# RobinChen121/Stochastic-Inventory

Hardware: NVIDIA B200
Metric: state-action-demand evaluations/s (fp64), full-horizon SDP solve (higher is better)
Workload: dtype f64

## Files before the change

stochastic-inventory_b200/csrc/kernel_lead.cuh:

```cuda
#pragma once
#include <cuda_runtime.h>

#include <cstdlib>

#include "dev_model.cuh"
#include "kernel_tiled.cuh"

namespace sdpb {

constexpr int kLeadYT = 4;

struct LeadArgs {
    int t, D, pmf_off;
    const double* Vn;
    double* Vt;
    int* Qt;
    long long lo, hi;
    long long row0;
    int NYT;
    int ny_tiles, nq2_tiles;
    int A, Apad, di_max, NR;
    int nthreads;
};

__device__ __forceinline__ long long lds_s64(unsigned shared_addr) {
    long long v;
    asm volatile("ld.shared.s64 %0, [%1];" : "=l"(v) : "r"(shared_addr));
    return v;
}

__device__ __forceinline__ double ldg_at(const char* base, long long byte_off) {
    return __ldg(reinterpret_cast<const double*>(base + byte_off));
}

__device__ __forceinline__ double lds_double(unsigned shared_addr) {
    double v;
    asm volatile("ld.shared.f64 %0, [%1];" : "=d"(v) : "r"(shared_addr));
    return v;
}

template <bool IS_MIN, bool LAST, int RQ, bool DEDUP>
__global__ void __launch_bounds__(256)
bi_lead_slab(const __grid_constant__ DevModel M, const __grid_constant__ LeadArgs a) {
    constexpr int YT = kLeadYT;
    extern __shared__ __align__(16) unsigned char smem_raw[];
    const int NYB = YT * a.NYT;
    const int D = a.D, A = a.A, Apad = a.Apad;
    double* slab = reinterpret_cast<double*>(smem_raw);
    const size_t slab_elems = (size_t)max(a.NR, NYB) * RQ * Apad;
    double* Lw = slab + slab_elems;
    double2* PP = reinterpret_cast<double2*>(Lw + ((a.NR + 1) & ~1));

    long long b = blockIdx.x;
    int q2_0 = 0;
    if (M.lead == 2) { q2_0 = (int)(b % a.nq2_tiles) * RQ; b /= a.nq2_tiles; }
    const int ytile = (int)(b % a.ny_tiles); b /= a.ny_tiles;
    const long long ix = DEDUP ? 0 : a.row0 + b;
    const int q1_0 = ytile * NYB;
    const long long y0 = ix + q1_0;
    const int n_levels = DEDUP ? (M.nI + M.nQ - 1) : M.nQ;

    const int tid = threadIdx.x;
    for (int j = tid; j < D; j += a.nthreads) PP[j] = make_double2(M.pmf_p[a.pmf_off + j], M.pmf_pg[a.pmf_off + j]);
    const bool lost = (M.flags & SDPB_F_LOST_SALES) != 0;
    const long long strideX = (M.lead == 2) ? (long long)M.nQ * M.nQ : (long long)M.nQ;
    for (int wi = tid; wi < a.NR; wi += a.nthreads) {
        const double lvl = M.inv_min + (double)(y0 - a.di_max + wi) * M.step;
        Lw[wi] = M.h * fmax(lvl, 0.0) + M.pen * fmax(-lvl, 0.0);
    }
    if (!LAST) {
// ... 382 lines not shown
    if (mn) { if (last) SDPB_COL_LAUNCH(true, true) else SDPB_COL_LAUNCH(true, false) }
    else    { if (last) SDPB_COL_LAUNCH(false, true) else SDPB_COL_LAUNCH(false, false) }
#undef SDPB_COL_LAUNCH
    if (e != cudaSuccess || cudaGetLastError() != cudaSuccess) return SDPB_ERR_CUDA;
    return SDPB_OK;
}

struct DevPeer { char* base0; unsigned long long stride; long long lo, hi; };

template <bool IS_MIN>
__global__ void __launch_bounds__(256)
merge_action_slices(const double* __restrict__ sv, const int* __restrict__ sa, int parts, long long n_local,
                    double* __restrict__ Vt, int* __restrict__ Qt, long long lo, const DevPeer* __restrict__ peers,
                    int n_peers, int t) {
    const long long i = (long long)blockIdx.x * blockDim.x + threadIdx.x;
    if (i >= n_local) return;
    double best = IS_MIN ? DBL_MAX : -DBL_MAX;
    int arg = kNoAction;
    for (int q = 0; q < parts; q++) {
        const double v = sv[(long long)q * n_local + i];
        const int av = sa[(long long)q * n_local + i];
        if (av != kNoAction && (IS_MIN ? (v < best) : (v > best))) { best = v; arg = av; }
    }
    Vt[i] = best;
    Qt[i] = arg == kNoAction ? -1 : arg;
    const long long idx = lo + i;
    for (int p = 0; p < n_peers; p++) {
        const DevPeer pr = peers[p];
        if (idx >= pr.lo && idx < pr.hi)
            reinterpret_cast<double*>(pr.base0 + (unsigned long long)(t - 1) * pr.stride)[idx] = best;
    }
}

struct Q2Args {
    int t, D, pmf_off;
    const double* VnT;
    double* Vt;
    int* Qt;
    long long lo, hi;
    long long f_begin, f_end;
    int n_chunks, tpx;
    int cs;
    double* slice_v;
    int* slice_a;
    int di_max, NRW;
    int parts;
    int n_peer;
    double* peer_v[2];
    long long peer_lo[2], peer_hi[2];
};

struct PeerStore { double* v; long long lo, hi; };

constexpr int kQ2YT = 8, kQ2PF = 2, kQ2PAD = kQ2PF + 1;

__global__ void transpose_q2a(const double* __restrict__ V, double* __restrict__ VT, int nQ, int row0) {
    __shared__ double tile[32][33];
    const long long base = (long long)(row0 + blockIdx.x) * nQ * nQ;
    const int c0 = blockIdx.y * 32, r0 = blockIdx.z * 32;
    for (int r = threadIdx.y; r < 32; r += 8) {
        const int row = r0 + r, c = c0 + threadIdx.x;
        if (row < nQ && c < nQ) tile[r][threadIdx.x] = V[base + (long long)row * nQ + c];
    }
    __syncthreads();
    for (int r = threadIdx.y; r < 32; r += 8) {
        const int row = c0 + r, c = r0 + threadIdx.x;
        if (row < nQ && c < nQ) VT[base + (long long)row * nQ + c] = tile[threadIdx.x][r];
    }
}

template <bool IS_MIN, bool LAST, int NT, int PARTS>
__global__ void __launch_bounds__(NT, 512 / NT)
bi_lead_q2(const __grid_constant__ DevModel M, const __grid_constant__ Q2Args a) {
    constexpr int YT = kQ2YT, PF = kQ2PF, W = YT + PF, PAD = kQ2PAD;
    extern __shared__ __align__(16) unsigned char smem_raw[];
    double2* WR = reinterpret_cast<double2*>(smem_raw);
    double2* PP = WR + a.NRW;
    const int D = a.D, nQ = M.nQ, tid = threadIdx.x;
    constexpr int cols = NT / PARTS;
    const int part = tid / cols, col = tid - part * cols;
    double* MV = reinterpret_cast<double*>(PP + D);
    int* MA = reinterpret_cast<int*>(MV + (size_t)(PARTS - 1) * YT * cols);
    const long long F0 = a.f_begin + (long long)blockIdx.x * cols;
    const long long x_first = F0 / a.tpx;
    const bool lost = (M.flags & SDPB_F_LOST_SALES) != 0;

    for (int j = tid; j < D; j += NT) PP[j] = make_double2(M.pmf_p[a.pmf_off + j], M.pmf_pg[a.pmf_off + j]);
    for (int wi = tid; wi < a.NRW; wi += NT) {
        const long long il = x_first - a.di_max - PAD + wi;
        const double lvl = M.inv_min + (double)il * M.step;
        long long is = il;
        if (lost) is = is > M.i_zero ? is : M.i_zero;
        is = is < M.nI - 1 ? is : M.nI - 1;
        is = is > 0 ? is : 0;
        WR[wi] = make_double2(M.h * fmax(lvl, 0.0) + M.pen * fmax(-lvl, 0.0),
// ... 78 lines not shown
        if (part > 0 || !any) return;
        for (int q = 0; q < PARTS - 1; q++) {
#pragma unroll
            for (int k = 0; k < YT; k++) {
                const double v = MV[(q * YT + k) * cols + col];
                const int av = MA[(q * YT + k) * cols + col];
                if (av != kNoAction && (IS_MIN ? (v < best[k]) : (v > best[k]))) { best[k] = v; arg[k] = av; }
            }
        }
    }
#pragma unroll
    for (int k = 0; k < YT; k++) {
        const long long idx = idx0 + (long long)k * nQ;
        if (l0 + k < nQ && idx >= a.lo && idx < a.hi) {
            a.Vt[idx] = best[k];
            a.Qt[idx] = arg[k] == kNoAction ? -1 : arg[k];
            for (int p = 0; p < a.n_peer; p++)
                if (idx >= a.peer_lo[p] && idx < a.peer_hi[p]) a.peer_v[p][idx] = best[k];
        }
    }
}

template <int IMM>
__device__ __forceinline__ double2 lds_double2_o(unsigned shared_addr) {
    double2 v;
    asm volatile("ld.shared.v2.f64 {%0, %1}, [%2+%3];" : "=d"(v.x), "=d"(v.y) : "r"(shared_addr), "n"(IMM));
    return v;
}

constexpr int kQ2mNC = 3;
constexpr int kQ2mPW = kQ2YT;
constexpr unsigned short kQ2mNoAction = 0xffff;

struct Q2mLayout { int NG; unsigned off_rg, off_gb, off_pz, off_bv, off_ba, off_mt; size_t smem; };

__host__ __device__ inline Q2mLayout q2m_layout(int NRW, int D, int NT, int cs) {
    Q2mLayout L;
    L.NG = (NT - 1) / cs + 2;
    const unsigned R = (unsigned)(D + kQ2YT - 1);
    unsigned o = (unsigned)(NRW + D) * 16u;
    L.off_rg = o; o += (unsigned)L.NG * R * 16u;
    L.off_gb = o; o += ((unsigned)L.NG * 4u + 15u) & ~15u;
    L.off_pz = o; o += ((R + kQ2YT - 1) * 8u + 15u) & ~15u;
    L.off_bv = o; o += (unsigned)(kQ2mNC * kQ2YT * NT) * 8u;
    L.off_ba = o; o += ((unsigned)(kQ2mNC * kQ2YT * NT) * 2u + 15u) & ~15u;
    L.off_mt = o; o += (unsigned)L.NG * R * 64u;
    L.smem = o;
    return L;
}

template <bool LAST, int KLO, int KHI, int PH, int VS, int IMM>
__device__ __forceinline__ void q2m_diag(double (&acc)[kQ2mNC][kQ2YT], unsigned mt, const double (&pw)[kQ2mPW],
                                         const double (&vb)[kQ2mNC][2]) {
    double mm[kQ2YT];
    if (KLO < 2 && KHI > 0) { const double2 t = lds_double2_o<IMM>(mt); mm[0] = t.x; mm[1] = t.y; }
    if (KLO < 4 && KHI > 2) { const double2 t = lds_double2_o<IMM + 16>(mt); mm[2] = t.x; mm[3] = t.y; }
    if (KLO < 6 && KHI > 4) { const double2 t = lds_double2_o<IMM + 32>(mt); mm[4] = t.x; mm[5] = t.y; }
    if (KLO < 8 && KHI > 6) { const double2 t = lds_double2_o<IMM + 48>(mt); mm[6] = t.x; mm[7] = t.y; }
#pragma unroll
    for (int k = KLO; k < KHI; k++)
#pragma unroll
        for (int c = 0; c < kQ2mNC; c++) {
            acc[c][k] += mm[k];
            if (!LAST) acc[c][k] += pw[(PH + k) % kQ2mPW] * vb[c][VS];
        }
}

template <int VS, int PS, int IMM>
__device__ __forceinline__ void q2m_refill(double (&pw)[kQ2mPW], double (&vb)[kQ2mNC][2], unsigned rg,
                                           const double* const (&cb)[kQ2mNC]) {
    const double2 r = lds_double2_o<IMM>(rg);
    if (PS >= 0) pw[PS < 0 ? 0 : PS] = r.x;
    const unsigned off = (unsigned)__double2loint(r.y);
#pragma unroll
    for (int c = 0; c < kQ2mNC; c++) vb[c][VS] = __ldg(cb[c] + off);
}

template <bool IS_MIN, bool LAST, int NT>
__global__ void __launch_bounds__(NT, 512 / NT)
bi_lead_q2m(const __grid_constant__ DevModel M, const __grid_constant__ Q2Args a) {
    constexpr int YT = kQ2YT, PAD = kQ2PAD, NC = kQ2mNC, PW = kQ2mPW;
    static_assert(YT == 8 && NC == 3 && PW == 8, "the diagonals below are written out for these sizes");
    static_assert(NT % 8 == 0, "the table builder keeps the slot index fixed per thread");
    extern __shared__ __align__(16) unsigned char smem_raw[];
    const int D = a.D, nQ = M.nQ, cs = a.cs, tid = threadIdx.x;
    const int R = D + YT - 1;
    const Q2mLayout L = q2m_layout(a.NRW, D, NT, cs);
    double2* WR = reinterpret_cast<double2*>(smem_raw);
    double2* PP = WR + a.NRW;
    double2* RG = reinterpret_cast<double2*>(smem_raw + L.off_rg);
    int* GB = reinterpret_cast<int*>(smem_raw + L.off_gb);
    double* PZ = reinterpret_cast<double*>(smem_raw + L.off_pz);
    double* BV = reinterpret_cast<double*>(smem_raw + L.off_bv);
    unsigned short* BA = reinterpret_cast<unsigned short*>(smem_raw + L.off_ba);
    double* MT = reinterpret_cast<double*>(smem_raw + L.off_mt);
    const int NG = L.NG;
    const long long F0 = a.f_begin + (long long)blockIdx.x * NT;
    const long long x_first = F0 / a.tpx;
    const long long G0 = F0 / cs;
    const bool lost = (M.flags & SDPB_F_LOST_SALES) != 0;

    for (int j = tid; j < D; j += NT) PP[j] = make_double2(M.pmf_p[a.pmf_off + j], M.pmf_pg[a.pmf_off + j]);
    for (int j = tid; j < R + YT - 1; j += NT) {
        const int jd = j - (YT - 1);
        PZ[j] = jd >= 0 && jd < D ? M.pmf_p[a.pmf_off + jd] : 0.0;
    }
    for (int wi = tid; wi < a.NRW; wi += NT) {
        const long long il = x_first - a.di_max - PAD + wi;
        const double lvl = M.inv_min + (double)il * M.step;
        long long is = il;
        if (lost) is = is > M.i_zero ? is : M.i_zero;
        is = is < M.nI - 1 ? is : M.nI - 1;
        is = is > 0 ? is : 0;
        WR[wi] = make_double2(M.h * fmax(lvl, 0.0) + M.pen * fmax(-lvl, 0.0),
                              __hiloint2double(0, (int)(is * nQ * nQ)));
    }
    for (int g = tid; g < NG; g += NT) {
        const long long G = G0 + g;
        const long long xg = G / a.n_chunks;
        const int chunk = (int)(G - xg * a.n_chunks);
        int wb = (int)(xg - x_first) + chunk * YT + (D - 1) + PAD;
        GB[g] = min(wb, a.NRW - YT);
    }
#pragma unroll
    for (int s2 = 0; s2 < NC * YT; s2++) { BV[s2 * NT + tid] = IS_MIN ? DBL_MAX : -DBL_MAX; BA[s2 * NT + tid] = kQ2mNoAction; }
    __syncthreads();
    for (int e = tid; e < NG * R; e += NT) {
        const int g = e / R, n = e - g * R;
        RG[e] = make_double2(n + 1 < D ? PP[n + 1].y : 0.0, WR[GB[g] + 5 - n].y);
    }

    const long long F = min(F0 + tid, a.f_end - 1);
    const long long x = F / a.tpx;
    const int f = (int)(F - x * a.tpx);
    const int chunk = f / cs, c0 = f - chunk * cs, l0 = chunk * YT;
    const int g_own = (int)(F / cs - G0);
    const long long idx0 = (x * nQ + l0) * nQ + c0;
    const long long idx_end = idx0 + (long long)(min(YT, nQ - l0) - 1) * nQ + (long long)((nQ - 1 - c0) / cs) * cs;
    const bool any = F0 + tid < a.f_end && idx_end >= a.lo && idx0 < a.hi;

    const unsigned wr_s = (unsigned)__cvta_generic_to_shared(WR);
    const unsigned pp_s = (unsigned)__cvta_generic_to_shared(PP);
    const unsigned rg0 = (unsigned)__cvta_generic_to_shared(RG) + (unsigned)(g_own * R) * 16u;
    const unsigned mt0 = (unsigned)__cvta_generic_to_shared(MT) + (unsigned)(g_own * R) * 64u;
    const unsigned bv_s = (unsigned)__cvta_generic_to_shared(BV) + (unsigned)tid * 8u;
    const unsigned ba_s = (unsigned)__cvta_generic_to_shared(BA) + (unsigned)tid * 2u;
    const int gb = (int)(x - x_first) + l0 + (D - 1) + PAD;
    const double* cb[NC];
#pragma unroll
    for (int c = 0; c < NC; c++) cb[c] = LAST ? nullptr : a.VnT + c0 + (c0 + c * cs < nQ ? c * cs : 0);
    const double vt = M.v_t[a.t - 1];

    const int n_sl = (int)gridDim.y, sl = (int)blockIdx.y;
    const int per_sl = (M.max_order_idx + n_sl) / n_sl;
    const int ai_begin = sl * per_sl, ai_end = min(M.max_order_idx + 1, ai_begin + per_sl);
#pragma unroll
    for (int c = 0; c < NC; c++) if (!LAST) cb[c] += (long long)ai_begin * nQ;
    for (int ai = ai_begin; ai < ai_end; ai++) {
        {
            const double av = (double)ai * M.step;
            const double fv = (av > 0.0 ? M.K : 0.0) + vt * av;
            for (int r = tid; r < NG * R; r += NT) {
                const int g = r / R, n = r - g * R;
                const double cst = fv + WR[GB[g] + (YT - 1) - n].x;
                double2* Mr = reinterpret_cast<double2*>(MT + (size_t)r * YT);
#pragma unroll
                for (int k = 0; k < YT; k += 2)
                    Mr[k / 2] = make_double2(PZ[n + k] * cst, PZ[n + k + 1] * cst);
            }
        }
        __syncthreads();
        if (any) {
            double acc[NC][YT];
#pragma unroll
            for (int c = 0; c < NC; c++)
#pragma unroll
                for (int k = 0; k < YT; k++) acc[c][k] = 0.0;
            if (D >= YT - 1) {
                double pw[PW], vb[NC][2];
                if (!LAST) {
                    pw[0] = lds_double(pp_s + 8u);
#pragma unroll
                    for (int n = 0; n < 2; n++) {
                        const unsigned off = (unsigned)__double2loint(lds_double(wr_s + (unsigned)(gb + 7 - n) * 16u + 8u));
#pragma unroll
                        for (int c = 0; c < NC; c++) vb[c][n] = __ldg(cb[c] + off);
                    }
                }
#define SDPB_Q2M_HEAD(N)                                                                              \
                q2m_diag<LAST, YT - 1 - (N), YT, (N) + 1, (N) & 1, (N) * 64>(acc, mt0, pw, vb);           \
                if (!LAST) q2m_refill<(N) & 1, (N) + 1, (N) * 16>(pw, vb, rg0, cb);
                SDPB_Q2M_HEAD(0) SDPB_Q2M_HEAD(1) SDPB_Q2M_HEAD(2) SDPB_Q2M_HEAD(3)
                SDPB_Q2M_HEAD(4) SDPB_Q2M_HEAD(5) SDPB_Q2M_HEAD(6)
#undef SDPB_Q2M_HEAD
#define SDPB_Q2M_FULL(U)                                                                              \
                q2m_diag<LAST, 0, YT, (U), ((U) + 1) & 1, (U) * 64>(acc, mt_run, pw, vb);                 \
                if (!LAST) q2m_refill<((U) + 1) & 1, (U), (U) * 16>(pw, vb, rg_run, cb);
                int n = YT - 1;
                unsigned mt_run = mt0 + (unsigned)n * 64u, rg_run = rg0 + (unsigned)n * 16u;
                for (; n + PW <= D; n += PW, mt_run += PW * 64u, rg_run += PW * 16u) {
                    SDPB_Q2M_FULL(0) SDPB_Q2M_FULL(1) SDPB_Q2M_FULL(2) SDPB_Q2M_FULL(3) SDPB_Q2M_FULL(4)
                    SDPB_Q2M_FULL(5) SDPB_Q2M_FULL(6) SDPB_Q2M_FULL(7)
                }
                if (n + 0 < D) { SDPB_Q2M_FULL(0) }
                if (n + 1 < D) { SDPB_Q2M_FULL(1) }
                if (n + 2 < D) { SDPB_Q2M_FULL(2) }
                if (n + 3 < D) { SDPB_Q2M_FULL(3) }
                if (n + 4 < D) { SDPB_Q2M_FULL(4) }
                if (n + 5 < D) { SDPB_Q2M_FULL(5) }
                if (n + 6 < D) { SDPB_Q2M_FULL(6) }
                if (n + 7 < D) { SDPB_Q2M_FULL(7) }
#undef SDPB_Q2M_FULL
                double pe[PW], ve[NC][2];
                if (!LAST) {
#pragma unroll
                    for (int m = 0; m < YT - 1; m++) pe[m] = lds_double(pp_s + (unsigned)(D - (YT - 1) + m) * 16u + 8u);
                    const bool odd = (D & 1) != 0;
#pragma unroll
                    for (int c = 0; c < NC; c++) {
                        ve[c][0] = odd ? vb[c][1] : vb[c][0];
                        ve[c][1] = odd ? vb[c][0] : vb[c][1];
                    }
                }
                const unsigned mt_d = mt0 + (unsigned)D * 64u, rg_d = rg0 + (unsigned)D * 16u;
#define SDPB_Q2M_TAIL(E)                                                                              \
                q2m_diag<LAST, 0, YT - 1 - (E), (E), (E) & 1, (E) * 64>(acc, mt_d, pe, ve);               \
                if (!LAST && (E) + 2 < YT - 1) q2m_refill<(E) & 1, -1, (E) * 16>(pe, ve, rg_d, cb);
                SDPB_Q2M_TAIL(0) SDPB_Q2M_TAIL(1) SDPB_Q2M_TAIL(2) SDPB_Q2M_TAIL(3)
                SDPB_Q2M_TAIL(4) SDPB_Q2M_TAIL(5) SDPB_Q2M_TAIL(6)
#undef SDPB_Q2M_TAIL
            } else {
                for (int n = 0; n < R; n++) {
                    double mm[YT], v[NC];
                    if (!LAST) {
                        const unsigned off = (unsigned)__double2loint(lds_double(wr_s + (unsigned)(gb + 7 - n) * 16u + 8u));
#pragma unroll
                        for (int c = 0; c < NC; c++) v[c] = __ldg(cb[c] + off);
                    }
#pragma unroll
                    for (int p = 0; p < YT / 2; p++) {
                        const double2 t = lds_double2(mt0 + (unsigned)n * 64u + (unsigned)p * 16u);
                        mm[2 * p] = t.x; mm[2 * p + 1] = t.y;
                    }
#pragma unroll
                    for (int k = 0; k < YT; k++) {
                        const int j = n - (YT - 1) + k;
                        if (j < 0 || j >= D) continue;
                        const double pg = LAST ? 0.0 : lds_double(pp_s + (unsigned)j * 16u + 8u);
#pragma unroll
                        for (int c = 0; c < NC; c++) {
                            acc[c][k] += mm[k];
                            if (!LAST) acc[c][k] += pg * v[c];
                        }
                    }
                }
            }
#pragma unroll
            for (int c = 0; c < NC; c++)
#pragma unroll
                for (int k = 0; k < YT; k++) {
                    const unsigned so = (unsigned)((c * YT + k) * NT);
                    const double bv = lds_double(bv_s + so * 8u);
                    if (IS_MIN ? (acc[c][k] < bv) : (acc[c][k] > bv)) {
                        asm volatile("st.shared.f64 [%0], %1;" ::"r"(bv_s + so * 8u), "d"(acc[c][k]) : "memory");
                        asm volatile("st.shared.u16 [%0], %1;" ::"r"(ba_s + so * 2u), "h"((unsigned short)ai) : "memory");
                    }
                }
        }
        __syncthreads();
#pragma unroll
        for (int c = 0; c < NC; c++) if (!LAST) cb[c] += nQ;
    }
    if (!any) return;
    unsigned ts;
    asm volatile("mov.u32 %0, %%tid.x;" : "=r"(ts));
    const long long Fs = min(F0 + (long long)ts, a.f_end - 1);
    const long long xs = Fs / a.tpx;
    const int fs = (int)(Fs - xs * a.tpx);
    const int cks = fs / cs, c0s = fs - cks * cs, l0s = cks * YT;
    const long long idx0s = (xs * nQ + l0s) * nQ + c0s;
#pragma unroll
    for (int c = 0; c < NC; c++) {
        if (c0s + c * cs >= nQ) break;
#pragma unroll
        for (int k = 0; k < YT; k++) {
            const long long idx = idx0s + (long long)k * nQ + c * cs;
            if (!(l0s + k < nQ && idx >= a.lo && idx < a.hi)) continue;
            const double best = BV[(c * YT + k) * NT + ts];
            const unsigned short ba = BA[(c * YT + k) * NT + ts];
            const int arg = ba == kQ2mNoAction ? kNoAction : (int)ba;
            if (n_sl > 1) {
                a.slice_v[(long long)sl * (a.hi - a.lo) + (idx - a.lo)] = best;
                a.slice_a[(long long)sl * (a.hi - a.lo) + (idx - a.lo)] = arg;
                continue;
            }
            a.Vt[idx] = best;
            a.Qt[idx] = arg == kNoAction ? -1 : arg;
            for (int p = 0; p < a.n_peer; p++)
                if (idx >= a.peer_lo[p] && idx < a.peer_hi[p]) a.peer_v[p][idx] = best;
        }
    }
}

struct Q2Plan {
    bool ok = false;
    int NT = 128, n_chunks = 0, tpx = 0, di_max = 0, NRW = 0;
    size_t smem = 0;
};

inline Q2Plan plan_q2(const sdpb_model& m, const DevModel& d, int D, const int* di) {
    Q2Plan P;
    if (m.cost_kind != SDPB_COST_BACKORDER || m.lead_time != 2) return P;
    for (int j = 0; j < D; j++)
        if (di[j] != di[0] + j) return P;
    if ((long long)d.nI * d.nQ * d.nQ >= 0x7fffffffLL) return P;
    P.n_chunks = (d.nQ + kQ2YT - 1) / kQ2YT;
    P.tpx = P.n_chunks * d.nQ;
    P.di_max = di[D - 1];
    const int dx_max = (P.NT + P.tpx - 1) / P.tpx + 1;
    P.NRW = P.n_chunks * kQ2YT + D + kQ2PAD + dx_max;
    P.smem = (size_t)(P.NRW + D) * 16 + (size_t)kQ2YT * P.NT * 12;
    P.ok = P.smem <= 96 * 1024;
    return P;
}

constexpr int kQ2MaxPeers = 2;

struct Q2Shape { bool shared; int parts, slices, cs, tpx, NRW; long long f_begin, f_end; Q2mLayout L; };

inline Q2Shape q2_shape(const Q2Plan& P, const DevModel& dm, int D, long long lo, long long hi, int sm_count) {
    Q2Shape S{};
    const long long per_x = (long long)dm.nQ * dm.nQ;
    const long long rows = (hi - 1) / per_x - lo / per_x + 1;
    const double waves = (double)(rows * P.tpx) / 32.0 / (16.0 * sm_count);
    S.parts = waves >= 6.0 ? 1 : (waves >= 3.0 ? 2 : 4);
    S.cs = (dm.nQ + kQ2mNC - 1) / kQ2mNC;
    const int tpx2 = P.n_chunks * S.cs;
    const int NRW2 = P.n_chunks * kQ2YT + D + kQ2PAD + (P.NT + tpx2 - 1) / tpx2 + 1;
    S.slices = 1;
    S.L = q2m_layout(NRW2, D, P.NT, S.cs);
    static const bool force_share = std::getenv("SDPB_Q2_SHARE") != nullptr;
    static const int force_split = [] { const char* e = std::getenv("SDPB_Q2_SPLIT"); return e ? std::atoi(e) : 0; }();
    if (force_split) {
        S.parts = force_split == 2 ? 2 : 4;
    } else if (S.L.smem <= 56 * 1024) {
        S.shared = true; S.parts = 1;
        const double ctas = (double)(rows * tpx2) / P.NT;
        const double w = ctas / (4.0 * sm_count);
        if (w < 8.0 && !force_share) S.slices = (int)std::min(8.0, std::ceil(8.0 / std::max(w, 0.01)));
        S.slices = std::max(1, std::min(S.slices, (dm.max_order_idx + 1) / 8));
        const int per = (dm.max_order_idx + S.slices) / S.slices;
        S.slices = (dm.max_order_idx + per) / per;
    }
    S.tpx = S.shared ? tpx2 : P.tpx;
    S.NRW = S.shared ? NRW2 : P.NRW;
    S.f_begin = (lo / per_x) * S.tpx;
    S.f_end = ((hi - 1) / per_x + 1) * S.tpx;
    return S;
}

inline int launch_q2(const Q2Plan& P, const Q2Shape& S, const DevModel& dm, int t, int D, int pmf_off, const double* Vn,
                     double* VnT, double* Vt, int* Qt, long long lo, long long hi, int row0, int row1, cudaStream_t stream,
                     const PeerStore* peers, int n_peers, double* slice_v, int* slice_a, size_t slice_cap,
                     const DevPeer* d_peers, int n_dev_peers) {
    if (hi <= lo) return SDPB_OK;
    const bool last = (Vn == nullptr), mn = dm.is_min != 0;
    if (!last) {
        const unsigned tiles = (unsigned)((dm.nQ + 31) / 32);
        transpose_q2a<<<dim3((unsigned)(row1 - row0), tiles, tiles), dim3(32, 8), 0, stream>>>(Vn, VnT, dm.nQ, row0);
    }
    const long long n_local = hi - lo;
    if (S.slices > 1 && (size_t)S.slices * (size_t)n_local > slice_cap) return SDPB_ERR_NOMEM;
    Q2Args a;
    a.t = t; a.D = D; a.pmf_off = pmf_off; a.VnT = last ? nullptr : VnT; a.Vt = Vt; a.Qt = Qt; a.lo = lo; a.hi = hi;
    a.n_chunks = P.n_chunks; a.tpx = S.tpx; a.di_max = P.di_max; a.NRW = S.NRW;
    a.f_begin = S.f_begin; a.f_end = S.f_end; a.parts = S.parts; a.cs = S.cs;
    a.slice_v = slice_v; a.slice_a = slice_a;
    a.n_peer = 0;
    for (int p = 0; p < kQ2MaxPeers; p++) { a.peer_v[p] = nullptr; a.peer_lo[p] = a.peer_hi[p] = 0; }
    if (S.slices == 1)
        for (int p = 0; p < n_peers && p < kQ2MaxPeers; p++) {
            a.peer_v[p] = peers[p].v; a.peer_lo[p] = peers[p].lo; a.peer_hi[p] = peers[p].hi;
            a.n_peer = p + 1;
        }
    const int cols = P.NT / a.parts;
    const Q2mLayout L = S.L;
    const bool shared = S.shared;
    cudaError_t e = cudaSuccess;
    const dim3 grid((unsigned)((a.f_end - a.f_begin + cols - 1) / cols), (unsigned)S.slices);
#define SDPB_Q2_LAUNCH(K, SMEM, GRID)                                                                  \
    {                                                                                                  \
        auto k = K;                                                                                    \
        if (SMEM > 48 * 1024) e = cudaFuncSetAttribute(k, cudaFuncAttributeMaxDynamicSharedMemorySize, (int)SMEM); \
        if (e == cudaSuccess) k<<<GRID, 128, SMEM, stream>>>(dm, a);                                   \
    }
#define SDPB_Q2_NT(MN, LS)                                                                             \
    if (shared) SDPB_Q2_LAUNCH((bi_lead_q2m<MN, LS, 128>), L.smem, grid)                               \
    else if (a.parts == 1) SDPB_Q2_LAUNCH((bi_lead_q2<MN, LS, 128, 1>), P.smem, grid.x)                \
    else if (a.parts == 2) SDPB_Q2_LAUNCH((bi_lead_q2<MN, LS, 128, 2>), P.smem, grid.x)                \
    else SDPB_Q2_LAUNCH((bi_lead_q2<MN, LS, 128, 4>), P.smem, grid.x)
    if (mn) { if (last) SDPB_Q2_NT(true, true) else SDPB_Q2_NT(true, false) }
    else    { if (last) SDPB_Q2_NT(false, true) else SDPB_Q2_NT(false, false) }
#undef SDPB_Q2_NT
#undef SDPB_Q2_LAUNCH
    if (e != cudaSuccess || cudaGetLastError() != cudaSuccess) return SDPB_ERR_CUDA;
    if (S.slices > 1) {
        const unsigned mb = (unsigned)((n_local + 255) / 256);
        if (mn) merge_action_slices<true><<<mb, 256, 0, stream>>>(slice_v, slice_a, S.slices, n_local, Vt + lo, Qt + lo, lo, d_peers, n_dev_peers, t);
        else merge_action_slices<false><<<mb, 256, 0, stream>>>(slice_v, slice_a, S.slices, n_local, Vt + lo, Qt + lo, lo, d_peers, n_dev_peers, t);
        if (cudaGetLastError() != cudaSuccess) return SDPB_ERR_CUDA;
// ... 6 lines not shown
```

stochastic-inventory_b200/csrc/sdpb200.cu:

```cuda
#include <cuda_runtime.h>

#include <algorithm>
#include <chrono>
#include <cmath>
#include <cstdio>
#include <cstring>
#include <mutex>
#include <string>
#include <vector>

#include <unistd.h>

#include "../../include/sdpb200.h"
#include "dev_model.cuh"
#include "kernel_generic.cuh"
#include "kernel_tiled.cuh"
#include "kernel_lead.cuh"
#include "kernel_cash.cuh"
#include "kernel_two_product.cuh"
#include "kernel_staff.cuh"
#include "kernel_collapsed.cuh"
#include "kernel_fused.cuh"
#include "microbench.cuh"

// ... 694 lines not shown
        else if (t == m.T) h->stats.fp64_ops += executed * (surv ? 2.0 + 3.0 / kCashR : 1.0 + 4.0 / (sh.wide ? kCashRLast : kCashR));
        else h->stats.fp64_ops += executed * (surv ? 2.0 : 3.0 + 2.0 / kCashR);
        break;
    }
    case SDPB_KERNEL_LEAD_Q2: {
        const Q2Plan qp = plan_q2(m, h->dm, D, h->pmf_di.data() + off);
        const Q2Shape shape = q2_shape(qp, h->dm, D, lo, hi, h->sm_count);
        int64_t rlo = 0, rhi = h->S;
        sdpb_shard_reads(h, &rlo, &rhi);
        const long long per_x = (long long)h->dm.nQ * h->dm.nQ;
        PeerStore ps[kQ2MaxPeers];
        int nps = 0;
        if (shape.slices > 1) {
            if (int e = grow_slice_scratch(h, (size_t)shape.slices * (size_t)(hi - lo), h->q2_slice_v, h->q2_slice_a,
                                           h->q2_slice_cap))
                return e;
            if (push) h->push_fused = true;
        } else if (push && h->peer.sends.size() <= (size_t)kQ2MaxPeers) {
            for (const PeerSend& sd : h->peer.sends) {
                const PeerInfo& pi = h->peer.info[sd.rank];
                char* base = h->peer.mapped[sd.rank] + pi.v_off0 + (size_t)(t - 1) * pi.v_stride;
                ps[nps++] = PeerStore{reinterpret_cast<double*>(base) - pi.vlo, sd.a, sd.b};
            }
            h->push_fused = true;
        }
        const bool merge_pushes = push && shape.slices > 1;
        rc = launch_q2(qp, shape, h->dm, t, D, off, Vn, h->dVT, Vt, Qt, lo, hi, (int)(rlo / per_x), (int)(rhi / per_x),
                       h->stream, ps, nps, h->q2_slice_v, h->q2_slice_a, h->q2_slice_cap,
                       merge_pushes ? (const DevPeer*)h->peer.d_peers : nullptr, merge_pushes ? (int)h->peer.sends.size() : 0);
        if (rc != SDPB_OK) return rc;
        const bool ran = hi > lo;
        if (!last) h->stats.launches++;
        if (ran && shape.slices > 1) h->stats.launches++;
        if (ran && shape.shared) { used = SDPB_KERNEL_LEAD_Q2M; h->stats.fp64_ops += ev_range * (last ? 1.0 : 3.0); }
        else h->stats.fp64_ops += ev_range * (last ? (1.0 + 2.0 * kQ2YT) / kQ2YT : (1.0 + 4.0 * kQ2YT) / kQ2YT);
        break;
    }
    case SDPB_KERNEL_LEAD_COL: {
        const ColPlan cp = plan_col(m, h->dm, D, h->pmf_di.data() + off, h->dedup);
        rc = h->dedup ? launch_col<true>(cp, h->dm, t, D, off, Vn, Vt, Qt, lo, hi, h->stream)
                      : launch_col<false>(cp, h->dm, t, D, off, Vn, Vt, Qt, lo, hi, h->stream);
        h->stats.fp64_ops += ev_range * (last ? (1.0 + 2.0 * kColYT) / kColYT : (1.0 + 4.0 * kColYT) / kColYT);
        break;
    }
    case SDPB_KERNEL_LEAD_SLAB: {
        const LeadPlan lp = plan_lead(m, h->dm, D, h->pmf_di.data() + off);
        rc = h->dedup ? launch_lead<true>(lp, h->dm, t, D, off, Vn, Vt, Qt, lo, hi, h->stream)
                      : launch_lead<false>(lp, h->dm, t, D, off, Vn, Vt, Qt, lo, hi, h->stream);
        const double q = 4.0 * lp.RQ;
        h->stats.fp64_ops += ev_range * (last ? (5.0 + q) / q : (5.0 + 3.0 * q) / q);
        break;
    }
    case SDPB_KERNEL_STAGED:
        rc = h->dedup ? launch_staged<true>(h, t, Vn, Vt, Qt, lo, hi) : launch_staged<false>(h, t, Vn, Vt, Qt, lo, hi);
        h->stats.fp64_ops += (double)(hi - lo) * (plain ? 1 : m.max_order_idx + 1) * D * (last ? 3.0 : 5.0);
        break;
    case SDPB_KERNEL_CASH_TAIL: {
        const CashTailPlan tp = plan_cash_tail(m, h->dm, D, h->pmf_d.data(), (int)h->pmf_d.size());
        rc = launch_cash_tail(tp, m, h->dm, t, D, off, Vn, Vt, Qt, lo, hi, h->stream);
        const int kd = m.cost_kind;
        const double body = kd == SDPB_COST_CASH_DEPOSIT ? 4.0 : kd == SDPB_COST_CASH_OVERDRAFT ? 2.0 : kd == SDPB_COST_CASH_OD_LIMIT ? 9.0 : 7.0;
        h->stats.fp64_ops += executed * (last ? body + 3.0 : body + 8.0);
        break;
    }
    case SDPB_KERNEL_CASH_ROW:
        rc = launch_cash_row(m, h->dm, t, D, off, Vn, Vt, Qt, lo, hi, h->stream);
        h->stats.fp64_ops += executed * (last ? 8.0 : 13.0);
        break;
// ... 1452 lines not shown
```

Before: 4434 billion.

## Interleave Q2M value columns and pack table-build offsets for vectorized loads

The transpose now permutes columns so the three cs-strided value columns a thread reads sit contiguously, letting one row pointer serve all three loads. The MT table builder uses precomputed packed offsets in RG instead of per-item division, the best-value buffer moves to double2, the layout is computed once on the host, and the first diagonal initializes accumulators instead of zeroing them. The out-of-range early skip (`any`) is removed, so all threads compute. This adds complexity and depends on the permuted transpose matching the kernel's index mapping.

```diff
diff --git a/stochastic-inventory_b200/csrc/kernel_lead.cuh b/stochastic-inventory_b200/csrc/kernel_lead.cuh
--- a/stochastic-inventory_b200/csrc/kernel_lead.cuh
+++ b/stochastic-inventory_b200/csrc/kernel_lead.cuh
@@ -36,6 +36,12 @@
 __device__ __forceinline__ double lds_double(unsigned shared_addr) {
     double v;
     asm volatile("ld.shared.f64 %0, [%1];" : "=d"(v) : "r"(shared_addr));
+    return v;
+}
+
+__device__ __forceinline__ unsigned lds_u32(unsigned shared_addr) {
+    unsigned v;
+    asm volatile("ld.shared.u32 %0, [%1];" : "=r"(v) : "r"(shared_addr));
     return v;
 }
 
@@ -484,6 +490,8 @@
     }
 }
 
+struct Q2mLayout { int NG; unsigned off_rg, off_gb, off_pz, off_bv, off_ba, off_mt; size_t smem; };
+
 struct Q2Args {
     int t, D, pmf_off;
     const double* VnT;
@@ -497,6 +505,8 @@
     int* slice_a;
     int di_max, NRW;
     int parts;
+    int per_sl;
+    Q2mLayout L;
     int n_peer;
     double* peer_v[2];
     long long peer_lo[2], peer_hi[2];
@@ -506,13 +516,24 @@
 
 constexpr int kQ2YT = 8, kQ2PF = 2, kQ2PAD = kQ2PF + 1;
 
-__global__ void transpose_q2a(const double* __restrict__ V, double* __restrict__ VT, int nQ, int row0) {
+__host__ __device__ inline int q2m_col_base(int c0, int cs, int nQ) {
+    return min(3 * c0, max(0, min(3 * (cs - 1), nQ - 2)));
+}
+
+__device__ __forceinline__ int q2m_col_at(int p, int cs, int nQ) {
+    if (cs == 0) return p;
+    const int bl = q2m_col_base(cs - 1, cs, nQ);
+    const int c0 = p >= bl ? cs - 1 : p / 3;
+    return c0 + (p - q2m_col_base(c0, cs, nQ)) * cs;
+}
+
+__global__ void transpose_q2a(const double* __restrict__ V, double* __restrict__ VT, int nQ, int row0, int cs) {
     __shared__ double tile[32][33];
     const long long base = (long long)(row0 + blockIdx.x) * nQ * nQ;
     const int c0 = blockIdx.y * 32, r0 = blockIdx.z * 32;
     for (int r = threadIdx.y; r < 32; r += 8) {
         const int row = r0 + r, c = c0 + threadIdx.x;
-        if (row < nQ && c < nQ) tile[r][threadIdx.x] = V[base + (long long)row * nQ + c];
+        if (row < nQ && c < nQ) tile[r][threadIdx.x] = V[base + (long long)q2m_col_at(row, cs, nQ) * nQ + c];
     }
     __syncthreads();
     for (int r = threadIdx.y; r < 32; r += 8) {
@@ -657,8 +678,6 @@
 constexpr int kQ2mPW = kQ2YT;
 constexpr unsigned short kQ2mNoAction = 0xffff;
 
-struct Q2mLayout { int NG; unsigned off_rg, off_gb, off_pz, off_bv, off_ba, off_mt; size_t smem; };
-
 __host__ __device__ inline Q2mLayout q2m_layout(int NRW, int D, int NT, int cs) {
     Q2mLayout L;
     L.NG = (NT - 1) / cs + 2;
@@ -666,7 +685,7 @@
     unsigned o = (unsigned)(NRW + D) * 16u;
     L.off_rg = o; o += (unsigned)L.NG * R * 16u;
     L.off_gb = o; o += ((unsigned)L.NG * 4u + 15u) & ~15u;
-    L.off_pz = o; o += ((R + kQ2YT - 1) * 8u + 15u) & ~15u;
+    L.off_pz = o; o += (R + 6u) * 16u;
     L.off_bv = o; o += (unsigned)(kQ2mNC * kQ2YT * NT) * 8u;
     L.off_ba = o; o += ((unsigned)(kQ2mNC * kQ2YT * NT) * 2u + 15u) & ~15u;
     L.off_mt = o; o += (unsigned)L.NG * R * 64u;
@@ -674,7 +693,7 @@
     return L;
 }
 
-template <bool LAST, int KLO, int KHI, int PH, int VS, int IMM>
+template <bool LAST, int KLO, int KHI, int PH, int VS, int IMM, bool FIRST = false>
 __device__ __forceinline__ void q2m_diag(double (&acc)[kQ2mNC][kQ2YT], unsigned mt, const double (&pw)[kQ2mPW],
                                          const double (&vb)[kQ2mNC][2]) {
     double mm[kQ2YT];
@@ -686,19 +705,20 @@
     for (int k = KLO; k < KHI; k++)
 #pragma unroll
         for (int c = 0; c < kQ2mNC; c++) {
-            acc[c][k] += mm[k];
+            if (FIRST && k == KLO) acc[c][k] = mm[k];
+            else acc[c][k] += mm[k];
             if (!LAST) acc[c][k] += pw[(PH + k) % kQ2mPW] * vb[c][VS];
         }
 }
 
 template <int VS, int PS, int IMM>
 __device__ __forceinline__ void q2m_refill(double (&pw)[kQ2mPW], double (&vb)[kQ2mNC][2], unsigned rg,
-                                           const double* const (&cb)[kQ2mNC]) {
+                                           const double* cb) {
     const double2 r = lds_double2_o<IMM>(rg);
     if (PS >= 0) pw[PS < 0 ? 0 : PS] = r.x;
-    const unsigned off = (unsigned)__double2loint(r.y);
-#pragma unroll
-    for (int c = 0; c < kQ2mNC; c++) vb[c][VS] = __ldg(cb[c] + off);
+    const double* row = cb + (unsigned)__double2loint(r.y);
+#pragma unroll
+    for (int c = 0; c < kQ2mNC; c++) vb[c][VS] = __ldg(row + c);
 }
 
 template <bool IS_MIN, bool LAST, int NT>
@@ -710,13 +730,13 @@
     extern __shared__ __align__(16) unsigned char smem_raw[];
     const int D = a.D, nQ = M.nQ, cs = a.cs, tid = threadIdx.x;
     const int R = D + YT - 1;
-    const Q2mLayout L = q2m_layout(a.NRW, D, NT, cs);
+    const Q2mLayout& L = a.L;
     double2* WR = reinterpret_cast<double2*>(smem_raw);
     double2* PP = WR + a.NRW;
     double2* RG = reinterpret_cast<double2*>(smem_raw + L.off_rg);
     int* GB = reinterpret_cast<int*>(smem_raw + L.off_gb);
-    double* PZ = reinterpret_cast<double*>(smem_raw + L.off_pz);
-    double* BV = reinterpret_cast<double*>(smem_raw + L.off_bv);
+    double2* PZ2 = reinterpret_cast<double2*>(smem_raw + L.off_pz);
+    double2* BV = reinterpret_cast<double2*>(smem_raw + L.off_bv);
     unsigned short* BA = reinterpret_cast<unsigned short*>(smem_raw + L.off_ba);
     double* MT = reinterpret_cast<double*>(smem_raw + L.off_mt);
     const int NG = L.NG;
@@ -726,9 +746,10 @@
     const bool lost = (M.flags & SDPB_F_LOST_SALES) != 0;
 
     for (int j = tid; j < D; j += NT) PP[j] = make_double2(M.pmf_p[a.pmf_off + j], M.pmf_pg[a.pmf_off + j]);
-    for (int j = tid; j < R + YT - 1; j += NT) {
-        const int jd = j - (YT - 1);
-        PZ[j] = jd >= 0 && jd < D ? M.pmf_p[a.pmf_off + jd] : 0.0;
+    for (int i = tid; i < R + YT - 2; i += NT) {
+        const int j0 = i - (YT - 1), j1 = j0 + 1;
+        PZ2[i] = make_double2(j0 >= 0 && j0 < D ? M.pmf_p[a.pmf_off + j0] : 0.0,
+                              j1 >= 0 && j1 < D ? M.pmf_p[a.pmf_off + j1] : 0.0);
     }
     for (int wi = tid; wi < a.NRW; wi += NT) {
         const long long il = x_first - a.di_max - PAD + wi;
@@ -748,80 +769,83 @@
         GB[g] = min(wb, a.NRW - YT);
     }
 #pragma unroll
-    for (int s2 = 0; s2 < NC * YT; s2++) { BV[s2 * NT + tid] = IS_MIN ? DBL_MAX : -DBL_MAX; BA[s2 * NT + tid] = kQ2mNoAction; }
+    for (int s2 = 0; s2 < NC * YT / 2; s2++) BV[s2 * NT + tid] = IS_MIN ? make_double2(DBL_MAX, DBL_MAX) : make_double2(-DBL_MAX, -DBL_MAX);
+#pragma unroll
+    for (int s2 = 0; s2 < NC * YT; s2++) BA[s2 * NT + tid] = kQ2mNoAction;
     __syncthreads();
     for (int e = tid; e < NG * R; e += NT) {
         const int g = e / R, n = e - g * R;
-        RG[e] = make_double2(n + 1 < D ? PP[n + 1].y : 0.0, WR[GB[g] + 5 - n].y);
-    }
+        const unsigned build = (unsigned)(GB[g] + (YT - 1) - n) * 16u | (unsigned)n << 20;
+        RG[e] = make_double2(n + 1 < D ? PP[n + 1].y : 0.0, __hiloint2double((int)build, __double2loint(WR[GB[g] + 5 - n].y)));
+    }
+    __syncthreads();
 
     const long long F = min(F0 + tid, a.f_end - 1);
     const long long x = F / a.tpx;
     const int f = (int)(F - x * a.tpx);
     const int chunk = f / cs, c0 = f - chunk * cs, l0 = chunk * YT;
     const int g_own = (int)(F / cs - G0);
-    const long long idx0 = (x * nQ + l0) * nQ + c0;
-    const long long idx_end = idx0 + (long long)(min(YT, nQ - l0) - 1) * nQ + (long long)((nQ - 1 - c0) / cs) * cs;
-    const bool any = F0 + tid < a.f_end && idx_end >= a.lo && idx0 < a.hi;
-
-    const unsigned wr_s = (unsigned)__cvta_generic_to_shared(WR);
+
     const unsigned pp_s = (unsigned)__cvta_generic_to_shared(PP);
-    const unsigned rg0 = (unsigned)__cvta_generic_to_shared(RG) + (unsigned)(g_own * R) * 16u;
     const unsigned mt0 = (unsigned)__cvta_generic_to_shared(MT) + (unsigned)(g_own * R) * 64u;
-    const unsigned bv_s = (unsigned)__cvta_generic_to_shared(BV) + (unsigned)tid * 8u;
-    const unsigned ba_s = (unsigned)__cvta_generic_to_shared(BA) + (unsigned)tid * 2u;
-    const int gb = (int)(x - x_first) + l0 + (D - 1) + PAD;
-    const double* cb[NC];
-#pragma unroll
-    for (int c = 0; c < NC; c++) cb[c] = LAST ? nullptr : a.VnT + c0 + (c0 + c * cs < nQ ? c * cs : 0);
-    const double vt = M.v_t[a.t - 1];
+    const double* cb = LAST ? nullptr : a.VnT + q2m_col_base(c0, cs, nQ);
+    const unsigned n_items = 4u * (unsigned)(NG * R);
+    const unsigned sm_s = (unsigned)__cvta_generic_to_shared(smem_raw);
+    const unsigned rg_s = (unsigned)__cvta_generic_to_shared(RG), pz_s = (unsigned)__cvta_generic_to_shared(PZ2);
+    const unsigned mt_s = (unsigned)__cvta_generic_to_shared(MT);
 
     const int n_sl = (int)gridDim.y, sl = (int)blockIdx.y;
-    const int per_sl = (M.max_order_idx + n_sl) / n_sl;
-    const int ai_begin = sl * per_sl, ai_end = min(M.max_order_idx + 1, ai_begin + per_sl);
-#pragma unroll
-    for (int c = 0; c < NC; c++) if (!LAST) cb[c] += (long long)ai_begin * nQ;
-    for (int ai = ai_begin; ai < ai_end; ai++) {
+    const int ai_begin = sl * a.per_sl;
+    if (!LAST) cb += (long long)ai_begin * nQ;
+    for (int ai = ai_begin;; ai++) {
+        unsigned sy;
+        asm volatile("mov.u32 %0, %%ctaid.y;" : "=r"(sy));
+        if (ai >= min(M.max_order_idx + 1, (int)(sy + 1) * a.per_sl)) break;
         {
+            double vt;
+            asm volatile("{ .reg .u64 g; cvta.to.global.u64 g, %1; ld.global.nc.f64 %0, [g]; }"
+                         : "=d"(vt) : "l"(M.v_t + (a.t - 1)));
             const double av = (double)ai * M.step;
             const double fv = (av > 0.0 ? M.K : 0.0) + vt * av;
-            for (int r = tid; r < NG * R; r += NT) {
-                const int g = r / R, n = r - g * R;
-                const double cst = fv + WR[GB[g] + (YT - 1) - n].x;
-                double2* Mr = reinterpret_cast<double2*>(MT + (size_t)r * YT);
-#pragma unroll
-                for (int k = 0; k < YT; k += 2)
-                    Mr[k / 2] = make_double2(PZ[n + k] * cst, PZ[n + k + 1] * cst);
+            unsigned tb;
+            asm volatile("mov.u32 %0, %%tid.x;" : "=r"(tb));
+            const unsigned pz_t = pz_s + (tb & 3u) * 32u;
+            unsigned rg_r = rg_s + 12u + (tb >> 2) * 16u;
+            unsigned mt_r = mt_s + tb * 16u;
+            for (unsigned r = tb; r < n_items; r += NT, mt_r += NT * 16u, rg_r += NT * 4u) {
+                const unsigned w = lds_u32(rg_r);
+                const double cst = fv + lds_double(sm_s + (w & 0xffffu));
+                const double2 p = lds_double2(pz_t + (w >> 16));
+                asm volatile("st.shared.v2.f64 [%0], {%1, %2};" ::"r"(mt_r),
+                             "d"(__dadd_rn(0.0, __dmul_rn(p.x, cst))), "d"(__dadd_rn(0.0, __dmul_rn(p.y, cst))) : "memory");
             }
         }
         __syncthreads();
-        if (any) {
+        {
+            const unsigned rg0 = rg_s + ((mt0 - mt_s) >> 2);
+            const unsigned u0_s = sm_s + lds_u32(rg0 + 12u);
             double acc[NC][YT];
-#pragma unroll
-            for (int c = 0; c < NC; c++)
-#pragma unroll
-                for (int k = 0; k < YT; k++) acc[c][k] = 0.0;
-            if (D >= YT - 1) {
+            if (D >= YT) {
                 double pw[PW], vb[NC][2];
                 if (!LAST) {
                     pw[0] = lds_double(pp_s + 8u);
 #pragma unroll
                     for (int n = 0; n < 2; n++) {
-                        const unsigned off = (unsigned)__double2loint(lds_double(wr_s + (unsigned)(gb + 7 - n) * 16u + 8u));
-#pragma unroll
-                        for (int c = 0; c < NC; c++) vb[c][n] = __ldg(cb[c] + off);
+                        const double* row = cb + (unsigned)__double2loint(lds_double(u0_s - (unsigned)n * 16u + 8u));
+#pragma unroll
+                        for (int c = 0; c < NC; c++) vb[c][n] = __ldg(row + c);
                     }
                 }
 #define SDPB_Q2M_HEAD(N)                                                                              \
-                q2m_diag<LAST, YT - 1 - (N), YT, (N) + 1, (N) & 1, (N) * 64>(acc, mt0, pw, vb);           \
-                if (!LAST) q2m_refill<(N) & 1, (N) + 1, (N) * 16>(pw, vb, rg0, cb);
+                q2m_diag<LAST, YT - 1 - (N), YT, ((N) + 1) % PW, (N) & 1, (N) * 64, true>(acc, mt0, pw, vb); \
+                if (!LAST) q2m_refill<(N) & 1, ((N) + 1) % PW, (N) * 16>(pw, vb, rg0, cb);
                 SDPB_Q2M_HEAD(0) SDPB_Q2M_HEAD(1) SDPB_Q2M_HEAD(2) SDPB_Q2M_HEAD(3)
-                SDPB_Q2M_HEAD(4) SDPB_Q2M_HEAD(5) SDPB_Q2M_HEAD(6)
+                SDPB_Q2M_HEAD(4) SDPB_Q2M_HEAD(5) SDPB_Q2M_HEAD(6) SDPB_Q2M_HEAD(7)
 #undef SDPB_Q2M_HEAD
 #define SDPB_Q2M_FULL(U)                                                                              \
-                q2m_diag<LAST, 0, YT, (U), ((U) + 1) & 1, (U) * 64>(acc, mt_run, pw, vb);                 \
-                if (!LAST) q2m_refill<((U) + 1) & 1, (U), (U) * 16>(pw, vb, rg_run, cb);
-                int n = YT - 1;
+                q2m_diag<LAST, 0, YT, ((U) + 1) % PW, (U) & 1, (U) * 64>(acc, mt_run, pw, vb);            \
+                if (!LAST) q2m_refill<(U) & 1, ((U) + 1) % PW, (U) * 16>(pw, vb, rg_run, cb);
+                int n = YT;
                 unsigned mt_run = mt0 + (unsigned)n * 64u, rg_run = rg0 + (unsigned)n * 16u;
                 for (; n + PW <= D; n += PW, mt_run += PW * 64u, rg_run += PW * 16u) {
                     SDPB_Q2M_FULL(0) SDPB_Q2M_FULL(1) SDPB_Q2M_FULL(2) SDPB_Q2M_FULL(3) SDPB_Q2M_FULL(4)
@@ -834,7 +858,6 @@
                 if (n + 4 < D) { SDPB_Q2M_FULL(4) }
                 if (n + 5 < D) { SDPB_Q2M_FULL(5) }
                 if (n + 6 < D) { SDPB_Q2M_FULL(6) }
-                if (n + 7 < D) { SDPB_Q2M_FULL(7) }
 #undef SDPB_Q2M_FULL
                 double pe[PW], ve[NC][2];
                 if (!LAST) {
@@ -855,12 +878,16 @@
                 SDPB_Q2M_TAIL(4) SDPB_Q2M_TAIL(5) SDPB_Q2M_TAIL(6)
 #undef SDPB_Q2M_TAIL
             } else {
+#pragma unroll
+                for (int c = 0; c < NC; c++)
+#pragma unroll
+                    for (int k = 0; k < YT; k++) acc[c][k] = 0.0;
                 for (int n = 0; n < R; n++) {
                     double mm[YT], v[NC];
                     if (!LAST) {
-                        const unsigned off = (unsigned)__double2loint(lds_double(wr_s + (unsigned)(gb + 7 - n) * 16u + 8u));
-#pragma unroll
-                        for (int c = 0; c < NC; c++) v[c] = __ldg(cb[c] + off);
+                        const double* row = cb + (unsigned)__double2loint(lds_double(u0_s - (unsigned)n * 16u + 8u));
+#pragma unroll
+                        for (int c = 0; c < NC; c++) v[c] = __ldg(row + c);
                     }
 #pragma unroll
                     for (int p = 0; p < YT / 2; p++) {
@@ -880,26 +907,33 @@
                     }
                 }
             }
+            unsigned to;
+            asm volatile("mov.u32 %0, %%tid.x;" : "=r"(to));
+            const unsigned bv_s = (unsigned)__cvta_generic_to_shared(BV) + to * 16u;
+            const unsigned ba_s = (unsigned)__cvta_generic_to_shared(BA) + to * 2u;
 #pragma unroll
             for (int c = 0; c < NC; c++)
 #pragma unroll
-                for (int k = 0; k < YT; k++) {
-                    const unsigned so = (unsigned)((c * YT + k) * NT);
-                    const double bv = lds_double(bv_s + so * 8u);
-                    if (IS_MIN ? (acc[c][k] < bv) : (acc[c][k] > bv)) {
-                        asm volatile("st.shared.f64 [%0], %1;" ::"r"(bv_s + so * 8u), "d"(acc[c][k]) : "memory");
-                        asm volatile("st.shared.u16 [%0], %1;" ::"r"(ba_s + so * 2u), "h"((unsigned short)ai) : "memory");
+                for (int k = 0; k < YT; k += 2) {
+                    const unsigned so = (unsigned)((c * YT + k) / 2 * NT) * 16u, sa = (unsigned)((c * YT + k) * NT) * 2u;
+                    const double2 bv = lds_double2(bv_s + so);
+                    if (IS_MIN ? (acc[c][k] < bv.x) : (acc[c][k] > bv.x)) {
+                        asm volatile("st.shared.f64 [%0], %1;" ::"r"(bv_s + so), "d"(acc[c][k]) : "memory");
+                        asm volatile("st.shared.u16 [%0], %1;" ::"r"(ba_s + sa), "h"((unsigned short)ai) : "memory");
+                    }
+                    if (IS_MIN ? (acc[c][k + 1] < bv.y) : (acc[c][k + 1] > bv.y)) {
+                        asm volatile("st.shared.f64 [%0], %1;" ::"r"(bv_s + so + 8u), "d"(acc[c][k + 1]) : "memory");
+                        asm volatile("st.shared.u16 [%0], %1;" ::"r"(ba_s + sa + (unsigned)NT * 2u), "h"((unsigned short)ai) : "memory");
                     }
                 }
         }
         __syncthreads();
-#pragma unroll
-        for (int c = 0; c < NC; c++) if (!LAST) cb[c] += nQ;
-    }
-    if (!any) return;
+        if (!LAST) cb += nQ;
+    }
     unsigned ts;
     asm volatile("mov.u32 %0, %%tid.x;" : "=r"(ts));
-    const long long Fs = min(F0 + (long long)ts, a.f_end - 1);
+    if (F0 + (long long)ts >= a.f_end) return;
+    const long long Fs = F0 + (long long)ts;
     const long long xs = Fs / a.tpx;
     const int fs = (int)(Fs - xs * a.tpx);
     const int cks = fs / cs, c0s = fs - cks * cs, l0s = cks * YT;
@@ -911,7 +945,7 @@
         for (int k = 0; k < YT; k++) {
             const long long idx = idx0s + (long long)k * nQ + c * cs;
             if (!(l0s + k < nQ && idx >= a.lo && idx < a.hi)) continue;
-            const double best = BV[(c * YT + k) * NT + ts];
+            const double best = reinterpret_cast<const double*>(BV)[((c * YT + k) / 2 * NT + ts) * 2 + (k & 1)];
             const unsigned short ba = BA[(c * YT + k) * NT + ts];
             const int arg = ba == kQ2mNoAction ? kNoAction : (int)ba;
             if (n_sl > 1) {
@@ -992,7 +1026,8 @@
     const bool last = (Vn == nullptr), mn = dm.is_min != 0;
     if (!last) {
         const unsigned tiles = (unsigned)((dm.nQ + 31) / 32);
-        transpose_q2a<<<dim3((unsigned)(row1 - row0), tiles, tiles), dim3(32, 8), 0, stream>>>(Vn, VnT, dm.nQ, row0);
+        transpose_q2a<<<dim3((unsigned)(row1 - row0), tiles, tiles), dim3(32, 8), 0, stream>>>(Vn, VnT, dm.nQ, row0,
+                                                                                               S.shared ? S.cs : 0);
     }
     const long long n_local = hi - lo;
     if (S.slices > 1 && (size_t)S.slices * (size_t)n_local > slice_cap) return SDPB_ERR_NOMEM;
@@ -1001,6 +1036,8 @@
     a.n_chunks = P.n_chunks; a.tpx = S.tpx; a.di_max = P.di_max; a.NRW = S.NRW;
     a.f_begin = S.f_begin; a.f_end = S.f_end; a.parts = S.parts; a.cs = S.cs;
     a.slice_v = slice_v; a.slice_a = slice_a;
+    a.per_sl = (dm.max_order_idx + S.slices) / S.slices;
+    a.L = S.L;
     a.n_peer = 0;
     for (int p = 0; p < kQ2MaxPeers; p++) { a.peer_v[p] = nullptr; a.peer_lo[p] = a.peer_hi[p] = 0; }
     if (S.slices == 1)
diff --git a/stochastic-inventory_b200/csrc/sdpb200.cu b/stochastic-inventory_b200/csrc/sdpb200.cu
--- a/stochastic-inventory_b200/csrc/sdpb200.cu
+++ b/stochastic-inventory_b200/csrc/sdpb200.cu
@@ -750,8 +750,10 @@
         const bool ran = hi > lo;
         if (!last) h->stats.launches++;
         if (ran && shape.slices > 1) h->stats.launches++;
-        if (ran && shape.shared) { used = SDPB_KERNEL_LEAD_Q2M; h->stats.fp64_ops += ev_range * (last ? 1.0 : 3.0); }
-        else h->stats.fp64_ops += ev_range * (last ? (1.0 + 2.0 * kQ2YT) / kQ2YT : (1.0 + 4.0 * kQ2YT) / kQ2YT);
+        if (ran && shape.shared) {
+            used = SDPB_KERNEL_LEAD_Q2M;
+            h->stats.fp64_ops += ev_range * ((last ? 1.0 : 3.0) - (D >= kQ2YT ? 1.0 / D : 0.0));
+        } else h->stats.fp64_ops += ev_range * (last ? (1.0 + 2.0 * kQ2YT) / kQ2YT : (1.0 + 4.0 * kQ2YT) / kQ2YT);
         break;
     }
     case SDPB_KERNEL_LEAD_COL: {
```

After: 4617 billion (median of 6 runs). +4.1%, better.

## Double-buffer the per-action shared-memory cost table to drop one barrier per action

Applied to the files above, without the earlier changes.

The shared-memory table of per-action cost terms (MT) is now double-buffered: the table for the next order quantity is built while the current one is consumed, so one __syncthreads per action iteration goes away. The table builder is also restructured so each thread writes a fixed pair of slots across rows, avoiding per-row division. If doubling the table would push shared memory past the 56 KB budget, the host falls back to a single buffer. The cost is more shared memory per block, which may reduce occupancy or change which planning path is chosen.

```diff
diff --git a/stochastic-inventory_b200/csrc/kernel_lead.cuh b/stochastic-inventory_b200/csrc/kernel_lead.cuh
--- a/stochastic-inventory_b200/csrc/kernel_lead.cuh
+++ b/stochastic-inventory_b200/csrc/kernel_lead.cuh
@@ -493,6 +493,7 @@
     long long f_begin, f_end;
     int n_chunks, tpx;
     int cs;
+    int mbufs;
     double* slice_v;
     int* slice_a;
     int di_max, NRW;
@@ -657,11 +658,12 @@
 constexpr int kQ2mPW = kQ2YT;
 constexpr unsigned short kQ2mNoAction = 0xffff;
 
-struct Q2mLayout { int NG; unsigned off_rg, off_gb, off_pz, off_bv, off_ba, off_mt; size_t smem; };
-
-__host__ __device__ inline Q2mLayout q2m_layout(int NRW, int D, int NT, int cs) {
+struct Q2mLayout { int NG, mbufs; unsigned off_rg, off_gb, off_pz, off_bv, off_ba, off_mt; size_t smem; };
+
+__host__ __device__ inline Q2mLayout q2m_layout(int NRW, int D, int NT, int cs, int mbufs) {
     Q2mLayout L;
     L.NG = (NT - 1) / cs + 2;
+    L.mbufs = mbufs;
     const unsigned R = (unsigned)(D + kQ2YT - 1);
     unsigned o = (unsigned)(NRW + D) * 16u;
     L.off_rg = o; o += (unsigned)L.NG * R * 16u;
@@ -669,7 +671,7 @@
     L.off_pz = o; o += ((R + kQ2YT - 1) * 8u + 15u) & ~15u;
     L.off_bv = o; o += (unsigned)(kQ2mNC * kQ2YT * NT) * 8u;
     L.off_ba = o; o += ((unsigned)(kQ2mNC * kQ2YT * NT) * 2u + 15u) & ~15u;
-    L.off_mt = o; o += (unsigned)L.NG * R * 64u;
+    L.off_mt = o; o += (unsigned)(mbufs * L.NG) * R * 64u;
     L.smem = o;
     return L;
 }
@@ -706,11 +708,11 @@
 bi_lead_q2m(const __grid_constant__ DevModel M, const __grid_constant__ Q2Args a) {
     constexpr int YT = kQ2YT, PAD = kQ2PAD, NC = kQ2mNC, PW = kQ2mPW;
     static_assert(YT == 8 && NC == 3 && PW == 8, "the diagonals below are written out for these sizes");
-    static_assert(NT % 8 == 0, "the table builder keeps the slot index fixed per thread");
+    static_assert(NT % 8 == 0, "the table builder keeps the slot pair fixed per thread");
     extern __shared__ __align__(16) unsigned char smem_raw[];
     const int D = a.D, nQ = M.nQ, cs = a.cs, tid = threadIdx.x;
     const int R = D + YT - 1;
-    const Q2mLayout L = q2m_layout(a.NRW, D, NT, cs);
+    const Q2mLayout L = q2m_layout(a.NRW, D, NT, cs, a.mbufs);
     double2* WR = reinterpret_cast<double2*>(smem_raw);
     double2* PP = WR + a.NRW;
     double2* RG = reinterpret_cast<double2*>(smem_raw + L.off_rg);
@@ -781,20 +783,29 @@
     const int ai_begin = sl * per_sl, ai_end = min(M.max_order_idx + 1, ai_begin + per_sl);
 #pragma unroll
     for (int c = 0; c < NC; c++) if (!LAST) cb[c] += (long long)ai_begin * nQ;
+
+    const unsigned mt_odd = a.mbufs == 2 ? (unsigned)(NG * R) * 64u : 0u;
+    auto build = [&](int ai) {
+        const double av = (double)ai * M.step;
+        const double fv = (av > 0.0 ? M.K : 0.0) + vt * av;
+        double* mt_a = MT + (ai & 1) * (mt_odd / 8u);
+        const int k = 2 * (tid % 4);
+        int g = tid / 4 / R, n = tid / 4 - g * R;
+        for (int r = tid / 4; r < NG * R; r += NT / 4) {
+            const double cst = fv + WR[GB[g] + (YT - 1) - n].x;
+            *reinterpret_cast<double2*>(mt_a + (size_t)r * YT + k) =
+                make_double2(PZ[n + k] * cst, PZ[n + k + 1] * cst);
+            for (n += NT / 4; n >= R; n -= R) g++;
+        }
+    };
+    if (mt_odd) {
+        build(ai_begin);
+        __syncthreads();
+    }
+    unsigned mt = mt0 + (ai_begin & 1) * mt_odd;
     for (int ai = ai_begin; ai < ai_end; ai++) {
-        {
-            const double av = (double)ai * M.step;
-            const double fv = (av > 0.0 ? M.K : 0.0) + vt * av;
-            for (int r = tid; r < NG * R; r += NT) {
-                const int g = r / R, n = r - g * R;
-                const double cst = fv + WR[GB[g] + (YT - 1) - n].x;
-                double2* Mr = reinterpret_cast<double2*>(MT + (size_t)r * YT);
-#pragma unroll
-                for (int k = 0; k < YT; k += 2)
-                    Mr[k / 2] = make_double2(PZ[n + k] * cst, PZ[n + k + 1] * cst);
-            }
-        }
-        __syncthreads();
+        if (!mt_odd || ai + 1 < ai_end) build(mt_odd ? ai + 1 : ai);
+        if (!mt_odd) __syncthreads();
         if (any) {
             double acc[NC][YT];
 #pragma unroll
@@ -813,7 +824,7 @@
                     }
                 }
 #define SDPB_Q2M_HEAD(N)                                                                              \
-                q2m_diag<LAST, YT - 1 - (N), YT, (N) + 1, (N) & 1, (N) * 64>(acc, mt0, pw, vb);           \
+                q2m_diag<LAST, YT - 1 - (N), YT, (N) + 1, (N) & 1, (N) * 64>(acc, mt, pw, vb);            \
                 if (!LAST) q2m_refill<(N) & 1, (N) + 1, (N) * 16>(pw, vb, rg0, cb);
                 SDPB_Q2M_HEAD(0) SDPB_Q2M_HEAD(1) SDPB_Q2M_HEAD(2) SDPB_Q2M_HEAD(3)
                 SDPB_Q2M_HEAD(4) SDPB_Q2M_HEAD(5) SDPB_Q2M_HEAD(6)
@@ -822,7 +833,7 @@
                 q2m_diag<LAST, 0, YT, (U), ((U) + 1) & 1, (U) * 64>(acc, mt_run, pw, vb);                 \
                 if (!LAST) q2m_refill<((U) + 1) & 1, (U), (U) * 16>(pw, vb, rg_run, cb);
                 int n = YT - 1;
-                unsigned mt_run = mt0 + (unsigned)n * 64u, rg_run = rg0 + (unsigned)n * 16u;
+                unsigned mt_run = mt + (unsigned)n * 64u, rg_run = rg0 + (unsigned)n * 16u;
                 for (; n + PW <= D; n += PW, mt_run += PW * 64u, rg_run += PW * 16u) {
                     SDPB_Q2M_FULL(0) SDPB_Q2M_FULL(1) SDPB_Q2M_FULL(2) SDPB_Q2M_FULL(3) SDPB_Q2M_FULL(4)
                     SDPB_Q2M_FULL(5) SDPB_Q2M_FULL(6) SDPB_Q2M_FULL(7)
@@ -847,7 +858,7 @@
                         ve[c][1] = odd ? vb[c][0] : vb[c][1];
                     }
                 }
-                const unsigned mt_d = mt0 + (unsigned)D * 64u, rg_d = rg0 + (unsigned)D * 16u;
+                const unsigned mt_d = mt + (unsigned)D * 64u, rg_d = rg0 + (unsigned)D * 16u;
 #define SDPB_Q2M_TAIL(E)                                                                              \
                 q2m_diag<LAST, 0, YT - 1 - (E), (E), (E) & 1, (E) * 64>(acc, mt_d, pe, ve);               \
                 if (!LAST && (E) + 2 < YT - 1) q2m_refill<(E) & 1, -1, (E) * 16>(pe, ve, rg_d, cb);
@@ -864,7 +875,7 @@
                     }
 #pragma unroll
                     for (int p = 0; p < YT / 2; p++) {
-                        const double2 t = lds_double2(mt0 + (unsigned)n * 64u + (unsigned)p * 16u);
+                        const double2 t = lds_double2(mt + (unsigned)n * 64u + (unsigned)p * 16u);
                         mm[2 * p] = t.x; mm[2 * p + 1] = t.y;
                     }
 #pragma unroll
@@ -893,6 +904,7 @@
                 }
         }
         __syncthreads();
+        mt = ai & 1 ? mt - mt_odd : mt + mt_odd;
 #pragma unroll
         for (int c = 0; c < NC; c++) if (!LAST) cb[c] += nQ;
     }
@@ -963,7 +975,8 @@
     const int tpx2 = P.n_chunks * S.cs;
     const int NRW2 = P.n_chunks * kQ2YT + D + kQ2PAD + (P.NT + tpx2 - 1) / tpx2 + 1;
     S.slices = 1;
-    S.L = q2m_layout(NRW2, D, P.NT, S.cs);
+    S.L = q2m_layout(NRW2, D, P.NT, S.cs, 2);
+    if (S.L.smem > 56 * 1024) S.L = q2m_layout(NRW2, D, P.NT, S.cs, 1);
     static const bool force_share = std::getenv("SDPB_Q2_SHARE") != nullptr;
     static const int force_split = [] { const char* e = std::getenv("SDPB_Q2_SPLIT"); return e ? std::atoi(e) : 0; }();
     if (force_split) {
@@ -999,7 +1012,7 @@
     Q2Args a;
     a.t = t; a.D = D; a.pmf_off = pmf_off; a.VnT = last ? nullptr : VnT; a.Vt = Vt; a.Qt = Qt; a.lo = lo; a.hi = hi;
     a.n_chunks = P.n_chunks; a.tpx = S.tpx; a.di_max = P.di_max; a.NRW = S.NRW;
-    a.f_begin = S.f_begin; a.f_end = S.f_end; a.parts = S.parts; a.cs = S.cs;
+    a.f_begin = S.f_begin; a.f_end = S.f_end; a.parts = S.parts; a.cs = S.cs; a.mbufs = S.L.mbufs;
     a.slice_v = slice_v; a.slice_a = slice_a;
     a.n_peer = 0;
     for (int p = 0; p < kQ2MaxPeers; p++) { a.peer_v[p] = nullptr; a.peer_lo[p] = a.peer_hi[p] = 0; }
```

Result: faster. 4434 billion before, 4495 billion after (median of 6 runs) (+1.4%).
